# PABannier/bark.cpp

Hardware: NVIDIA H100
Metric: audio sec/sec (inverse RTF), bark-small f16, batch 1 per GPU, semantic->coarse->fine->encodec (higher is better)
Workload: dtype f16 weights/operands, f32 accumulate (reference arithmetic)

## Files before the change

bark.cpp_b200/__init__.py:

```python
from __future__ import annotations

import ctypes as C
import os

import numpy as np

_HERE = os.path.dirname(os.path.abspath(__file__))
LIB_PATH = os.path.join(_HERE, "libbark_b200.so")

PROGRESS_CB = C.CFUNCTYPE(None, C.c_void_p, C.c_int, C.c_int, C.c_void_p)


class BarkContextParams(C.Structure):
    _fields_ = [
        ("verbosity", C.c_int), ("temp", C.c_float), ("fine_temp", C.c_float), ("min_eos_p", C.c_float),
        ("sliding_window_size", C.c_int32), ("max_coarse_history", C.c_int32), ("sample_rate", C.c_int32),
        ("target_bandwidth", C.c_int32), ("cls_token_id", C.c_int32), ("sep_token_id", C.c_int32),
        ("n_steps_text_encoder", C.c_int32), ("text_pad_token", C.c_int32), ("text_encoding_offset", C.c_int32),
        ("semantic_rate_hz", C.c_float), ("semantic_pad_token", C.c_int32), ("semantic_vocab_size", C.c_int32),
        ("semantic_infer_token", C.c_int32), ("coarse_rate_hz", C.c_float), ("coarse_infer_token", C.c_int32),
        ("coarse_semantic_pad_token", C.c_int32), ("n_coarse_codebooks", C.c_int32), ("n_fine_codebooks", C.c_int32),
        ("codebook_size", C.c_int32), ("progress_callback", PROGRESS_CB), ("progress_callback_user_data", C.c_void_p),
    ]


class BarkStatistics(C.Structure):
    _fields_ = [("t_load_us", C.c_int64), ("t_eval_us", C.c_int64), ("t_semantic_us", C.c_int64), ("t_coarse_us", C.c_int64),
                ("t_fine_us", C.c_int64), ("n_sample_semantic", C.c_int32), ("n_sample_coarse", C.c_int32), ("n_sample_fine", C.c_int32)]


EXPORTS = [
    "bark_context_default_params", "bark_load_model", "bark_generate_audio", "bark_get_audio_data", "bark_get_audio_data_size",
    "bark_get_load_time", "bark_get_eval_time", "bark_reset_statistics", "bark_model_quantize", "bark_free",
    "bark_b200_set_device", "bark_b200_version", "bark_b200_gpt_eval", "bark_b200_fine_eval", "bark_b200_encodec_decode",
    "bark_b200_sample", "bark_b200_sample_rows", "bark_b200_reseed", "bark_b200_tokenize", "bark_b200_forward_text_encoder",
    "bark_b200_forward_coarse_encoder", "bark_b200_forward_fine_encoder", "bark_b200_get_tokens", "bark_b200_set_tokens",
    "bark_b200_get_stats", "bark_b200_get_hparams", "bark_b200_kernel_launches", "bark_b200_layernorm_fallbacks",
    "bark_b200_profile_enable", "bark_b200_profile_report", "bark_b200_io_counters", "bark_b200_decode_timing",
    "bark_b200_shard_init", "bark_b200_shard_connect", "bark_b200_shard_nvlink_bytes",
    "bark_b200_fast_mode", "bark_b200_fast_gemm", "bark_b200_fast_attention", "bark_b200_parity_attention",
    "bark_b200_generate_batch", "bark_b200_batch_audio", "bark_b200_batch_tokens", "bark_b200_gpt_eval_slot", "bark_b200_gpt_step_batch",
    "ggml_time_init", "ggml_time_us", "ggml_time_ms", "ggml_init", "ggml_free",
]

_lib = None


def lib() -> C.CDLL:
    global _lib
    if _lib is not None:
        return _lib
    if not os.path.exists(LIB_PATH):
        raise RuntimeError(f"{LIB_PATH} is missing: build the CUDA extension first (python -c 'import __graft_entry__ as g; g.build()'). "
                           "There is no CPU fallback.")
    L = C.CDLL(LIB_PATH)
    vp, i32p, f32p = C.c_void_p, C.c_void_p, C.c_void_p
    L.bark_context_default_params.restype = BarkContextParams
    L.bark_load_model.restype = vp
    L.bark_load_model.argtypes = [C.c_char_p, BarkContextParams, C.c_uint32]
    L.bark_generate_audio.restype = C.c_bool
    L.bark_generate_audio.argtypes = [vp, C.c_char_p, C.c_int]
    L.bark_get_audio_data.restype = C.POINTER(C.c_float)
    L.bark_get_audio_data.argtypes = [vp]
# ... 31 lines not shown
    L.bark_b200_kernel_launches.restype = C.c_ulonglong
    L.bark_b200_layernorm_fallbacks.restype = C.c_uint
    L.bark_b200_layernorm_fallbacks.argtypes = [vp]
    L.bark_b200_profile_enable.argtypes = [C.c_int]
    L.bark_b200_profile_report.restype = C.c_int
    L.bark_b200_profile_report.argtypes = [C.c_char_p, C.c_int]
    L.bark_b200_io_counters.argtypes = [C.POINTER(C.c_ulonglong), C.POINTER(C.c_ulonglong), C.c_int]
    L.bark_b200_decode_timing.restype = C.c_int
    L.bark_b200_decode_timing.argtypes = [vp, C.c_void_p, C.c_int]
    L.bark_b200_shard_init.restype = C.c_int
    L.bark_b200_shard_init.argtypes = [vp, C.c_int, C.c_int, vp]
    L.bark_b200_shard_connect.restype = C.c_int
    L.bark_b200_shard_connect.argtypes = [vp, vp]
    L.bark_b200_shard_nvlink_bytes.restype = C.c_ulonglong
    L.bark_b200_shard_nvlink_bytes.argtypes = [vp, C.c_int]
    L.bark_b200_fast_mode.restype = C.c_int
    L.bark_b200_fast_mode.argtypes = [vp]
    L.bark_b200_fast_gemm.restype = C.c_int
    L.bark_b200_fast_gemm.argtypes = [vp, vp, vp, C.c_int, C.c_int, C.c_int, C.c_int, C.c_int]
    L.bark_b200_fast_attention.restype = C.c_int
    L.bark_b200_fast_attention.argtypes = [vp, vp, vp, vp, C.c_int, C.c_int, C.c_int]
    L.bark_b200_parity_attention.restype = C.c_int
    L.bark_b200_parity_attention.argtypes = [vp, vp, vp, vp] + [C.c_int] * 7
    L.bark_b200_generate_batch.restype = C.c_bool
    L.bark_b200_generate_batch.argtypes = [vp, C.POINTER(C.c_char_p), C.POINTER(C.c_uint32), C.c_int, C.c_int]
    L.bark_b200_batch_audio.restype = C.c_int
    L.bark_b200_batch_audio.argtypes = [vp, C.c_int, f32p, C.c_int]
    L.bark_b200_batch_tokens.restype = C.c_int
    L.bark_b200_batch_tokens.argtypes = [vp, C.c_int, C.c_int, i32p, C.c_int]
    L.bark_b200_gpt_eval_slot.restype = C.c_int
    L.bark_b200_gpt_eval_slot.argtypes = [vp, C.c_int, C.c_int, i32p, C.c_int, C.POINTER(C.c_int), C.c_int, f32p]
    L.bark_b200_gpt_step_batch.restype = C.c_int
    L.bark_b200_gpt_step_batch.argtypes = [vp, C.c_int, C.c_int, i32p, i32p, i32p, f32p]
    L.ggml_time_us.restype = C.c_int64
    _lib = L
    return L


def _p(a: np.ndarray):
    return a.ctypes.data_as(C.c_void_p)


class Bark:

    def __init__(self, model_path: str, seed: int = 0, n_steps_text_encoder: int | None = None, temp=None, fine_temp=None,
                 min_eos_p=None, device: int | None = None, progress=None):
# ... 212 lines not shown
def fast_attention(q: np.ndarray, k: np.ndarray, v: np.ndarray, n_head: int) -> np.ndarray:
    q, k, v = (np.ascontiguousarray(a, np.float16) for a in (q, k, v))
    n, E = q.shape
    out = np.zeros((n, E), np.float16)
    if not lib().bark_b200_fast_attention(_p(q), _p(k), _p(v), _p(out), n, E, n_head):
        raise RuntimeError("bark_b200_fast_attention failed")
    return out


ATTN_PATHS = {"auto": 0, "fused": 1, "tiled": 2}


def parity_attention(q: np.ndarray, k: np.ndarray, v: np.ndarray, n_head: int, n_past: int = 0, causal: bool = False, path: str = "auto") -> np.ndarray:
    q, k, v = (np.ascontiguousarray(a, np.float32) for a in (q, k, v))
    N, E = q.shape
    n_kv = k.shape[0]
    assert k.shape == v.shape == (n_kv, E), (q.shape, k.shape, v.shape)
    out = np.zeros((N, E), np.float32)
    if not lib().bark_b200_parity_attention(_p(q), _p(k), _p(v), _p(out), N, n_kv, n_past, E, n_head, int(causal), ATTN_PATHS[path]):
        raise RuntimeError("bark_b200_parity_attention failed")
    return out


def kernel_launches() -> int:
    return int(lib().bark_b200_kernel_launches())


def profile_enable(on: bool):
    lib().bark_b200_profile_enable(int(on))


def profile_report() -> dict:
    import json
    n = lib().bark_b200_profile_report(None, 0)
    buf = C.create_string_buffer(n + 16)
    lib().bark_b200_profile_report(buf, n + 16)
    return json.loads(buf.value.decode())


def io_counters(reset: bool = False):
    a, b = C.c_ulonglong(0), C.c_ulonglong(0)
    lib().bark_b200_io_counters(C.byref(a), C.byref(b), int(reset))
    return a.value, b.value
```

bark.cpp_b200/csrc/bark_api.cu:

```cuda
#include "../../include/bark_b200.h"
#include "context.h"
#include "gpt_kernels.h"

#include <algorithm>
#include <cmath>
#include <cstring>

using namespace bark;

namespace {

thread_local int g_device_override = -1;
bool quiet() { static const bool q = [] { const char * e = getenv("BARK_B200_QUIET"); return e && *e && *e != '0'; }(); return q; }

inline bool is_alpha(unsigned char c) { return (c >= 'a' && c <= 'z') || (c >= 'A' && c <= 'Z'); }
inline bool is_digit(unsigned char c) { return c >= '0' && c <= '9'; }
inline bool is_punct(unsigned char c) { return c > 32 && c < 127 && !is_alpha(c) && !is_digit(c); }

char fold_accent(unsigned char second) {
    const unsigned cp = 0xC0u + (second - 0x80u);
    const bool lower = cp >= 0xE0;
    const unsigned up = lower ? cp - 0x20 : cp;
    char base = 0;
    if (up >= 0xC0 && up <= 0xC5) base = 'A';
// ... 916 lines not shown
    BARK_CUDA_CHECK(cudaMalloc(&dq, (size_t) N * E * 4)); BARK_CUDA_CHECK(cudaMalloc(&dk, (size_t) n_kv * E * 4));
    BARK_CUDA_CHECK(cudaMalloc(&dv, (size_t) n_kv * E * 4)); BARK_CUDA_CHECK(cudaMalloc(&dout, (size_t) N * E * 4));
    BARK_CUDA_CHECK(cudaMalloc(&dsc, (size_t) H * N * n_kv * 4));
    BARK_CUDA_CHECK(cudaMemcpy(dq, q, (size_t) N * E * 4, cudaMemcpyHostToDevice)); BARK_CUDA_CHECK(cudaMemcpy(dk, k, (size_t) n_kv * E * 4, cudaMemcpyHostToDevice));
    BARK_CUDA_CHECK(cudaMemcpy(dv, v, (size_t) n_kv * E * 4, cudaMemcpyHostToDevice));
    BARK_CUDA_CHECK(cudaMemset(dout, 0xff, (size_t) N * E * 4));
    if (path == ATTN_TILED) {
        int dev = 0, n_sm = 0;
        BARK_CUDA_CHECK(cudaGetDevice(&dev)); BARK_CUDA_CHECK(cudaDeviceGetAttribute(&n_sm, cudaDevAttrMultiProcessorCount, dev));
        if (N > attn_tiled_max_rows(H, n_sm)) return 0;
    }
    attention(dq, dk, dv, N, n_kv, n_past, E, H, causal != 0, dsc, dout, W_Q4_0, E, 0, (AttnPath) path);
    BARK_CUDA_CHECK(cudaGetLastError());
    const cudaError_t e = cudaDeviceSynchronize();
    if (e != cudaSuccess) { fprintf(stderr, "bark_b200_parity_attention: %s\n", cudaGetErrorString(e)); return 0; }
    BARK_CUDA_CHECK(cudaMemcpy(out, dout, (size_t) N * E * 4, cudaMemcpyDeviceToHost));
    return 1;
}
extern "C" int bark_b200_parity_attention(const float * q, const float * k, const float * v, float * out, int N, int n_kv, int n_past, int E, int H, int causal,
                                          int path) {
    return guarded((int) 0, [&] { return bark_b200_parity_attention_impl(q, k, v, out, N, n_kv, n_past, E, H, causal, path); });
}

extern "C" bool bark_b200_generate_batch(struct bark_context * ctx, const char * const * texts, const uint32_t * seeds, int n, int n_threads) {
    (void) n_threads;
    return guarded(false, [&] { return generate_batch(ctx, texts, seeds, n); });
}
extern "C" int bark_b200_batch_audio(struct bark_context * ctx, int i, float * out, int cap) {
    if (!ctx || i < 0 || i >= (int) ctx->batch.results.size()) return -1;
    const std::vector<float> & a = ctx->batch.results[(size_t) i].audio;
    if (out) memcpy(out, a.data(), sizeof(float) * std::min(a.size(), (size_t) std::max(cap, 0)));
    return (int) a.size();
}
extern "C" int bark_b200_batch_tokens(struct bark_context * ctx, int i, int stage, int32_t * out, int cap) {
    if (!ctx || i < 0 || i >= (int) ctx->batch.results.size()) return -1;
    return copy_tokens(ctx->batch.results[(size_t) i], stage, out, cap);
}
static int bark_b200_gpt_eval_slot_impl(struct bark_context * ctx, int which, int slot, const int32_t * tokens, int n, int * n_past, int merge_ctx, float * logits_out) {
    if (!ctx || which < 0 || which > 1 || slot < 0 || slot >= kMaxBatch || !tokens || !n_past || !logits_out) return 0;
    BARK_CUDA_CHECK(cudaSetDevice(ctx->device));
    if (!ensure_batch_slots(ctx, slot + 1)) return 0;
    return gpt_eval(ctx, *pick(ctx, which), tokens, n, n_past, merge_ctx != 0, logits_out, 0, 0, ctx->batch.k[which][slot], ctx->batch.v[which][slot]) ? 1 : 0;
}
extern "C" int bark_b200_gpt_eval_slot(struct bark_context * ctx, int which, int slot, const int32_t * tokens, int n, int * n_past, int merge_ctx, float * logits_out) {
    return guarded((int) 0, [&] { return bark_b200_gpt_eval_slot_impl(ctx, which, slot, tokens, n, n_past, merge_ctx, logits_out); });
}
// ... 26 lines not shown
```

bark.cpp_b200/csrc/gemm_kernels.cu:

```cuda
#include "epilogue.cuh"
#include "gpt_kernels.h"

#include <algorithm>
#include <string.h>

namespace bark {

namespace {

__device__ __forceinline__ uint32_t smem_u32(const void * p) { return (uint32_t) __cvta_generic_to_shared(p); }
__device__ __forceinline__ void mbar_init(uint32_t bar, uint32_t count) { asm volatile("mbarrier.init.shared::cta.b64 [%0], %1;" ::"r"(bar), "r"(count)); }
__device__ __forceinline__ void mbar_expect_tx(uint32_t bar, uint32_t bytes) { asm volatile("mbarrier.arrive.expect_tx.shared::cta.b64 _, [%0], %1;" ::"r"(bar), "r"(bytes) : "memory"); }
__device__ __forceinline__ void mbar_wait(uint32_t bar, uint32_t parity) {
    asm volatile(
        "{\n\t.reg .pred p;\n\t"
        "WAIT_%=:\n\t"
        "mbarrier.try_wait.parity.shared::cta.b64 p, [%0], %1;\n\t"
        "@p bra DONE_%=;\n\t"
        "bra WAIT_%=;\n\t"
        "DONE_%=:\n\t}" ::"r"(bar), "r"(parity) : "memory");
}
__device__ __forceinline__ void mbar_arrive(uint32_t bar) { asm volatile("mbarrier.arrive.shared::cta.b64 _, [%0];" ::"r"(bar) : "memory"); }
__device__ __forceinline__ void tma_bulk_g2s(uint32_t dst, const void * src, uint32_t bytes, uint32_t bar) {
    asm volatile("cp.async.bulk.shared::cluster.global.mbarrier::complete_tx::bytes [%0], [%1], %2, [%3];" ::"r"(dst), "l"(src), "r"(bytes), "r"(bar) : "memory");
}

template <int N, int MASK>
__device__ __forceinline__ void butterfly_stage(float (&r)[64], bool upper) {
#pragma unroll
    for (int i = 0; i < N / 2; i++) {
        const float keep = upper ? r[i + N / 2] : r[i];
        const float send = upper ? r[i] : r[i + N / 2];
        r[i] = __fadd_rn(keep, __shfl_xor_sync(0xffffffffu, send, MASK));
    }
}
__device__ __forceinline__ int butterfly_reduce64(float (&r)[64], int lane) {
    butterfly_stage<64, 16>(r, (lane & 16) != 0);
    butterfly_stage<32, 8>(r, (lane & 8) != 0);
    butterfly_stage<16, 4>(r, (lane & 4) != 0);
    butterfly_stage<8, 1>(r, (lane & 1) != 0);
    butterfly_stage<4, 2>(r, (lane & 2) != 0);
    return ((lane & 16) << 1) | ((lane & 8) << 1) | ((lane & 4) << 1) | ((lane & 1) << 2) | (lane & 2);
}

constexpr int kBM = 32, kBO = 16, kStages = 4;
constexpr int kStageBytes = (kBM + kBO) * 512;

template <typename T> struct QuadOp;
template <> struct QuadOp<__half> {
    typedef uint2 V;
    static constexpr int kGroupsPerStage = 2;
    __device__ __forceinline__ static float elem(const uint2 & u, int c) {
        const uint32_t w = c < 2 ? u.x : u.y;
        const __half2 h = *reinterpret_cast<const __half2 *>(&w);
        return (c & 1) ? __high2float(h) : __low2float(h);
    }
};
template <> struct QuadOp<float> {
    typedef uint4 V;
    static constexpr int kGroupsPerStage = 1;
    __device__ __forceinline__ static float elem(const uint4 & u, int c) { return __uint_as_float(c == 0 ? u.x : c == 1 ? u.y : c == 2 ? u.z : u.w); }
};

}

template <typename T>
__global__ void __launch_bounds__(256, 2) lane_gemm_tiled_kernel(const T * __restrict__ Wg, int K, int w_gs, int O, const T * __restrict__ act, int act_gs, int M, MatmulEpilogue ep) {
    typedef typename QuadOp<T>::V QV;
    constexpr int GPS = QuadOp<T>::kGroupsPerStage;
    constexpr int kRowB = kGmGroup * sizeof(T);
    extern __shared__ __align__(128) unsigned char smem[];
    const uint32_t full = smem_u32(smem + kStages * kStageBytes);
    int * const cnt = reinterpret_cast<int *>(smem + kStages * kStageBytes + kStages * 8);
    const int tid = threadIdx.x, lane = tid & 31, warp = tid >> 5;
    const int wm = warp >> 1, wo = warp & 1;
    const int nsteps = K >> 5;
    const int ngroups = (nsteps + 3) >> 2;
    const int nstages = (ngroups + GPS - 1) / GPS;
    const int tiles_o = (O + kBO - 1) / kBO, tiles_m = (M + kBM - 1) / kBM, n_tiles = tiles_o * tiles_m;
    const int my_tiles = ((int) blockIdx.x < n_tiles) ? (n_tiles - 1 - (int) blockIdx.x) / (int) gridDim.x + 1 : 0;
    const int total_steps = my_tiles * nstages;

    if (tid == 0) {
        for (int s = 0; s < kStages; s++) { mbar_init(full + s * 8, 1); cnt[s] = 0; }
        asm volatile("fence.mbarrier_init.release.cluster;" ::: "memory");
    }
    __syncthreads();
    auto issue = [&](int step) {
        const int ti = step / nstages, sg = step - ti * nstages;
        const int tile = blockIdx.x + ti * gridDim.x;
        const int m0 = (tile / tiles_o) * kBM, o0 = (tile % tiles_o) * kBO;
        const int slot = step % kStages;
        const uint32_t bar = full + slot * 8;
        const int g0 = sg * GPS, ng = min(GPS, ngroups - g0);
        mbar_expect_tx(bar, (uint32_t)(ng * (kBM + kBO) * kRowB));
        const uint32_t dst = smem_u32(smem + (size_t) slot * kStageBytes);
        for (int j = 0; j < ng; j++) {
            tma_bulk_g2s(dst + j * (kBM + kBO) * kRowB, act + (size_t)(g0 + j) * act_gs + (size_t) m0 * kGmGroup, kBM * kRowB, bar);
            tma_bulk_g2s(dst + j * (kBM + kBO) * kRowB + kBM * kRowB, Wg + (size_t)(g0 + j) * w_gs + (size_t) o0 * kGmGroup, kBO * kRowB, bar);
        }
    };
    if (tid == 0) for (int s0 = 0; s0 < kStages && s0 < total_steps; s0++) issue(s0);

    int step = 0;
    for (int ti = 0; ti < my_tiles; ti++) {
        const int tile = blockIdx.x + ti * gridDim.x;
        const int m0 = (tile / tiles_o) * kBM, o0 = (tile % tiles_o) * kBO;
        float acc[64];
#pragma unroll
        for (int i = 0; i < 64; i++) acc[i] = 0.0f;
        for (int sg = 0; sg < nstages; sg++, step++) {
            const int slot = step % kStages;
            mbar_wait(full + slot * 8, (uint32_t)(step / kStages) & 1);
            const unsigned char * st = smem + (size_t) slot * kStageBytes;
#pragma unroll
            for (int j = 0; j < GPS; j++) {
                const int g = sg * GPS + j;
                if (g < ngroups) {
                    const int steps = min(4, nsteps - g * 4);
                    const unsigned char * ga = st + j * (kBM + kBO) * kRowB + lane * sizeof(QV), * gw = ga + kBM * kRowB;
                    QV pa[8], pw[8];
#pragma unroll
                    for (int mi = 0; mi < 8; mi++) pa[mi] = *reinterpret_cast<const QV *>(ga + (wm * 8 + mi) * kRowB);
#pragma unroll
                    for (int oi = 0; oi < 8; oi++) pw[oi] = *reinterpret_cast<const QV *>(gw + (wo * 8 + oi) * kRowB);
#pragma unroll
                    for (int c = 0; c < 4; c++) {
                        if (c < steps) {
                            float af[8], wf[8];
#pragma unroll
                            for (int mi = 0; mi < 8; mi++) af[mi] = QuadOp<T>::elem(pa[mi], c);
#pragma unroll
                            for (int oi = 0; oi < 8; oi++) wf[oi] = QuadOp<T>::elem(pw[oi], c);
#pragma unroll
                            for (int mi = 0; mi < 8; mi++)
#pragma unroll
                                for (int oi = 0; oi < 8; oi++) acc[mi * 8 + oi] = __fmaf_rn(wf[oi], af[mi], acc[mi * 8 + oi]);
                        }
                    }
                }
            }
            __syncwarp();
            if (lane == 0) {
                __threadfence_block();
                if (atomicAdd_block(&cnt[slot], 1) == 7) {
                    cnt[slot] = 0;
                    __threadfence_block();
                    asm volatile("fence.proxy.async.shared::cta;" ::: "memory");
                    if (step + kStages < total_steps) issue(step + kStages);
                }
            }
        }
        const int base = butterfly_reduce64(acc, lane);
        const int m = m0 + wm * 8 + (base >> 3), o = o0 + wo * 8 + (base & 7);
        if (m < M) {
            if (o < O) matmul_epilogue(ep, m, o, acc[0]);
            if (o + 1 < O) matmul_epilogue(ep, m, o + 1, acc[1]);
        }
    }
}

void lane_gemm_tiled(const DMat & W, const void * act, int act_gs, int rows, const MatmulEpilogue & ep, cudaStream_t s) {
    const size_t smem = (size_t) kStages * kStageBytes + kStages * 8 + kStages * 4 + 64;
    int dev = 0, n_sm = 0;
    BARK_CUDA_CHECK(cudaGetDevice(&dev));
    BARK_CUDA_CHECK(cudaDeviceGetAttribute(&n_sm, cudaDevAttrMultiProcessorCount, dev));
    static std::atomic<unsigned long long> configured{0};
    if (first_use_on_this_device(configured)) {
        BARK_CUDA_CHECK(cudaFuncSetAttribute(lane_gemm_tiled_kernel<__half>, cudaFuncAttributeMaxDynamicSharedMemorySize, (int) smem));
        BARK_CUDA_CHECK(cudaFuncSetAttribute(lane_gemm_tiled_kernel<float>, cudaFuncAttributeMaxDynamicSharedMemorySize, (int) smem));
    }
    if (!W.p_gm) { fprintf(stderr, "bark_b200: matrix has no group-major copy for the tiled mat-mul\n"); throw std::runtime_error("unsupported configuration (see the message above)"); }
    const int n_tiles = ((W.n_out + kBO - 1) / kBO) * ((rows + kBM - 1) / kBM);
    const int grid = min(n_tiles, 2 * n_sm);
    const int w_gs = W.o_pad * kGmGroup;
    if (W.type == W_F16) BARK_LAUNCH((lane_gemm_tiled_kernel<__half>), grid, 256, smem, s, (const __half *) W.p_gm, W.K, w_gs, W.n_out, (const __half *) act, act_gs, rows, ep);
    else                 BARK_LAUNCH((lane_gemm_tiled_kernel<float>), grid, 256, smem, s, (const float *) W.p_gm, W.K, w_gs, W.n_out, (const float *) act, act_gs, rows, ep);
}

constexpr int kAttnQ = 32, kAttnKT = 64, kAttnVK = 512, kAttnVW = 16;
constexpr int kAttnVLd = kAttnVW + 4;

__host__ __device__ inline int attn_ld(int n_kv) { return ((n_kv + 31) & ~31) + 1; }
__host__ __device__ inline int attn_ring_off(int n_kv) { return (kAttnQ * attn_ld(n_kv) + 3) & ~3; }

namespace {
__device__ __forceinline__ void cp_async_16(void * dst, const float * src) { asm volatile("cp.async.cg.shared.global [%0], [%1], 16;" ::"r"(smem_u32(dst)), "l"(src) : "memory"); }
__device__ __forceinline__ void cp_async_commit() { asm volatile("cp.async.commit_group;" ::: "memory"); }
__device__ __forceinline__ void cp_async_wait_prev() { asm volatile("cp.async.wait_group 1;" ::: "memory"); }
}

template <int DSTEPS>
__global__ void __launch_bounds__(256, 1) attn_fused_kernel(const float * __restrict__ Q, const float * __restrict__ Kc, const float * __restrict__ Vc,
                                                            int N, int n_kv, int n_past, int E, float scale, int causal,
                                                            void * __restrict__ act, int wt, int Kp) {
    constexpr int D = DSTEPS * 32;
    extern __shared__ __align__(16) float sm[];
    const int tid = threadIdx.x, lane = tid & 31, warp = tid >> 5;
    const int h = blockIdx.y, q0 = blockIdx.x * kAttnQ;
    const int ld = attn_ld(n_kv);
// ... 239 lines not shown
```

bark.cpp_b200/csrc/gpt_kernels.h:

```cpp
#pragma once
#include "model.h"

namespace bark {

enum EpiMode : int { EPI_STORE = 0, EPI_RESID = 1, EPI_GELU_ACT = 2, EPI_QKV = 3 };

struct MatmulEpilogue {
    int mode = EPI_STORE;
    float * out = nullptr; int ldo = 0;
    float * k_out = nullptr, * v_out = nullptr;
    int n_peer = 0; float * k_peer[7] = {nullptr}, * v_peer[7] = {nullptr};
    void * act_out = nullptr; int act_wt = 0, act_Kp = 0;
    const __half * gelu_tab = nullptr;
};

void permute_to_li(const void * src_rowmajor, void * dst_li, int n_out, int K, WType t, cudaStream_t s);
void permute_to_gm(const void * src_rowmajor, void * dst_gm, int n_out, int o_pad, int K, WType t, cudaStream_t s);

void gpt_embed_causal(const GPTModel & m, const int32_t * d_tok, int N, int n_past, bool merge, float * x, cudaStream_t s, const int32_t * d_pos = nullptr);
void gpt_embed_fine(const GPTModel & m, const int32_t * d_ids, int nn, float * x, cudaStream_t s, int row0 = 0, int rows = 1024);

void layernorm_act(const float * x, int rows, int E, const float * g, const float * b, void * act, WType wt, int Kp,
                   unsigned * fallback_counter, cudaStream_t s);

void lane_matmul(const DMat & W, const void * act, int act_gs, int rows, const MatmulEpilogue & ep, cudaStream_t s);

enum AttnPath : int { ATTN_AUTO = 0, ATTN_FUSED = 1, ATTN_TILED = 2 };
int  attn_tiled_max_rows(int H, int n_sm);
void attention(const float * Q, const float * Kc, const float * Vc, int N, int n_kv, int n_past, int E, int H, bool causal,
               float * scores, void * act, WType wt, int Kp, cudaStream_t s, AttnPath path = ATTN_AUTO);

struct BatchKV { float * k[8], * v[8]; };
void attention_batch(const float * Q, const float * Kst, const float * Vst, const BatchKV & kv, const int32_t * d_pos, int B, int max_kv, int E, int H,
                     float * scores, void * act, WType wt, int Kp, cudaStream_t s);

void q4_split(const void * raw_blocks, size_t n_blocks, void * qs, void * scales, cudaStream_t s);
void q4_set_scratch(void * q8, void * q8_scales);
void q4_matmul(const DMat & W, const void * act_f32, int ld_act, int rows, const MatmulEpilogue & ep, cudaStream_t s);

bool   qx_supported(WType t);
size_t qx_block_bytes(WType t);
void   qx_split(const void * raw_blocks, size_t n_blocks, WType t, void * qs, void * qh, void * d, void * m, cudaStream_t s);
void   qx_set_scratch(void * q8, void * q8_scales, void * q8_sums);
void   qx_embed_causal(const GPTModel & m, const int32_t * d_tok, int N, int n_past, bool merge, float * x, cudaStream_t s, const int32_t * d_pos);
void   qx_embed_fine(const GPTModel & m, const int32_t * d_ids, int nn, float * x, cudaStream_t s);
void   qx_matmul(const DMat & W, const void * act_f32, int ld_act, int rows, const MatmulEpilogue & ep, cudaStream_t s);

void lane_gemm_tiled(const DMat & W, const void * act, int act_gs, int rows, const MatmulEpilogue & ep, cudaStream_t s);

enum { FEPI_F32 = 0, FEPI_RESID = 1, FEPI_GELU16 = 2, FEPI_QKV16 = 4 };
struct FastEpi {
    int mode = FEPI_F32;
    float * out32 = nullptr; __half * out16 = nullptr; int ldo = 0;
    __half * vt = nullptr; int vt_ld = 0, v_col0 = 0;
};
int  fast_gemm(const __half * A, int lda, const __half * W, int ldw, int M, int N, int K, const FastEpi & ep, int n_sm, int bn, cudaStream_t s);
bool fast_attention(const __half * qk, int ldq, int k_col0, const __half * vt, int n, int E, int H, __half * out, cudaStream_t s);
void fast_layernorm(const float * x, int rows, int E, const float * g, const float * b, __half * out, cudaStream_t s);

constexpr int kDecodeReplicas = 8;
struct DecodePhase { const void * w; int n_out, row_bytes, K, pad; const void * ws; };
struct DecodeLayerVec { const float * ln_1_g, * ln_1_b, * ln_2_g, * ln_2_b; };
struct DecodeArgs {
    const DecodePhase * phases;
    const DecodeLayerVec * layer_vecs;
    const void * wte; const float * wpe; const float * ln_f_g, * ln_f_b; const __half * gelu_tab;
    float * mem_k, * mem_v;
    unsigned long long * gx, * gq, * gk, * gv, * gatt, * gff, * gscores;
    float * logits;
    unsigned tag_base; unsigned * ln_fallbacks;
    unsigned long long * timing;
// ... 13 lines not shown
```

bark.cpp_b200/csrc/loader.cu:

```cuda
#include "context.h"
#include "codec_kernels.h"
#include "gpt_kernels.h"

#include <cmath>
#include <cstring>
#include <fstream>

namespace bark {

static const uint32_t kMagic = 0x67676d6c;

void * ctx_alloc(bark_context * ctx, size_t bytes) {
    void * p = nullptr;
    BARK_CUDA_CHECK(cudaMalloc(&p, bytes ? bytes : 16));
    ctx->device_allocs.push_back(p);
    return p;
}

namespace {

template <typename T> bool rd(std::ifstream & f, T & v) { f.read(reinterpret_cast<char *>(&v), sizeof(T)); return (bool) f; }

size_t type_bytes(int ttype, size_t nel) {
    switch (ttype) {
// ... 105 lines not shown
                const size_t n_blocks = h.nel / 32;
                d.n_out = s.ne1; d.K = s.ne0; d.Kp = d.K; d.type = m.wtype;
                d.p = ctx_alloc(ctx, n_blocks * (m.wtype == W_Q8_0 ? 32 : 16)); d.scales = ctx_alloc(ctx, n_blocks * 2);
                d.mins = ctx_alloc(ctx, n_blocks * 2); d.qh = ctx_alloc(ctx, n_blocks * 4);
                qx_split(raw, n_blocks, m.wtype, d.p, d.qh, d.scales, d.mins, ctx->stream);
                BARK_CUDA_CHECK(cudaStreamSynchronize(ctx->stream));
                BARK_CUDA_CHECK(cudaFree(raw));
                continue;
            }
            if (m.wtype == W_Q4_0) {
                const size_t n_blocks = h.nel / 32;
                d.n_out = s.ne1; d.K = s.ne0; d.Kp = d.K; d.type = W_Q4_0;
                d.p = ctx_alloc(ctx, n_blocks * 16); d.scales = ctx_alloc(ctx, n_blocks * 2);
                q4_split(raw, n_blocks, d.p, d.scales, ctx->stream);
                BARK_CUDA_CHECK(cudaStreamSynchronize(ctx->stream));
                BARK_CUDA_CHECK(cudaFree(raw));
                if (ctx->params.verbosity == HIGH) printf("%48s - [%5d, %5d], type = %d, %6.2f MB\n", h.name.c_str(), h.ne[0], h.ne[1], h.ttype, bytes / 1024.0 / 1024.0);
                continue;
            }
            d.n_out = s.ne1; d.K = s.ne0; d.type = m.wtype; d.Kp = li_padded_k(d.K, m.wtype == W_F16 ? 2 : 4);
            d.p = ctx_alloc(ctx, (size_t) d.n_out * d.Kp * (m.wtype == W_F16 ? 2 : 4));
            permute_to_li(raw, d.p, d.n_out, d.K, m.wtype, ctx->stream);
            if (s.gm) {
                d.o_pad = (d.n_out + 15) / 16 * 16;
                const size_t gm_bytes = (size_t) gm_groups(d.K) * d.o_pad * kGmGroup * (m.wtype == W_F16 ? 2 : 4);
                d.p_gm = ctx_alloc(ctx, gm_bytes);
                permute_to_gm(raw, d.p_gm, d.n_out, d.o_pad, d.K, m.wtype, ctx->stream);
            }
            BARK_CUDA_CHECK(cudaStreamSynchronize(ctx->stream));
            if (ctx->fast_mode && !causal && m.wtype == W_F16) { d.p_rm = raw; ctx->device_allocs.push_back(raw); }
            else BARK_CUDA_CHECK(cudaFree(raw));
        } else {
            void * raw = upload_raw(ctx, f, bytes, host, true);
            if (!raw) return false;
            if (s.kind == Slot::TABLE) *s.table = raw; else *s.vec = (float *) raw;
        }
        if (ctx->params.verbosity == HIGH) printf("%48s - [%5d, %5d], type = %d, %6.2f MB\n", h.name.c_str(), h.ne[0], h.ne[1], h.ttype, bytes / 1024.0 / 1024.0);
    }
    for (auto & kv : slots) {
        const Slot & s = kv.second;
        const bool present = s.kind == Slot::MATRIX ? s.mat->p != nullptr : s.kind == Slot::TABLE ? *s.table != nullptr : *s.vec != nullptr;
        if (!present) { fprintf(stderr, "%s: tensor '%s' missing from the %s model\n", __func__, kv.first.c_str(), what); return false; }
    }
    if (causal) {
        const size_t n = (size_t) m.n_layer * m.block_size * E;
        m.mem_k = (float *) ctx_alloc(ctx, n * 4); m.mem_v = (float *) ctx_alloc(ctx, n * 4);
        BARK_CUDA_CHECK(cudaMemsetAsync(m.mem_k, 0, n * 4, ctx->stream)); BARK_CUDA_CHECK(cudaMemsetAsync(m.mem_v, 0, n * 4, ctx->stream));
// ... 157 lines not shown
```

include/bark_b200.h:

```cpp
#pragma once
#include "bark.h"

#ifdef __cplusplus
extern "C" {
#endif

BARK_API void bark_b200_set_device(int cuda_device);
BARK_API const char * bark_b200_version(void);

BARK_API int  bark_b200_gpt_eval(struct bark_context * ctx, int which, const int32_t * tokens, int n, int * n_past, int merge_ctx, float * logits_out);
BARK_API int  bark_b200_fine_eval(struct bark_context * ctx, const int32_t * in_buffer, int nn, float * logits_out);
BARK_API int  bark_b200_encodec_decode(struct bark_context * ctx, const int32_t * codes, int n_frames, float * out, int out_cap);
BARK_API int  bark_b200_sample(struct bark_context * ctx, int which, const float * logits, int n, float temp, float * eos_p);
BARK_API int  bark_b200_sample_rows(struct bark_context * ctx, const float * logits , int n, int rows, float temp, int32_t * tokens_out,
                                     float * eos_p_out );
BARK_API void bark_b200_reseed(struct bark_context * ctx, uint32_t seed);
BARK_API void bark_b200_tokenize(struct bark_context * ctx, const char * text, int32_t * out513);

BARK_API bool bark_b200_forward_text_encoder(struct bark_context * ctx, int n_threads);
BARK_API bool bark_b200_forward_coarse_encoder(struct bark_context * ctx, int n_threads);
BARK_API bool bark_b200_forward_fine_encoder(struct bark_context * ctx, int n_threads);

BARK_API int  bark_b200_get_tokens(struct bark_context * ctx, int stage, int32_t * out, int cap);
BARK_API void bark_b200_set_tokens(struct bark_context * ctx, int stage, const int32_t * in, int n);
// ... 5 lines not shown
BARK_API void bark_b200_profile_enable(int on);
BARK_API int  bark_b200_profile_report(char * buf, int cap);
BARK_API void bark_b200_io_counters(unsigned long long * h2d_bytes, unsigned long long * d2h_bytes, int reset);
BARK_API int  bark_b200_decode_timing(struct bark_context * ctx, unsigned long long * out, int n);


BARK_API int  bark_b200_shard_init(struct bark_context * ctx, int rank, int world, void * handle_out);
BARK_API int  bark_b200_shard_connect(struct bark_context * ctx, const void * all_handles);
BARK_API unsigned long long bark_b200_shard_nvlink_bytes(struct bark_context * ctx, int reset);

BARK_API bool bark_b200_generate_batch(struct bark_context * ctx, const char * const * texts, const uint32_t * seeds, int n, int n_threads);
BARK_API int  bark_b200_batch_audio(struct bark_context * ctx, int i, float * out, int cap);
BARK_API int  bark_b200_batch_tokens(struct bark_context * ctx, int i, int stage, int32_t * out, int cap);
BARK_API int  bark_b200_gpt_eval_slot(struct bark_context * ctx, int which, int slot, const int32_t * tokens, int n, int * n_past, int merge_ctx, float * logits_out);
BARK_API int  bark_b200_gpt_step_batch(struct bark_context * ctx, int which, int B, const int32_t * slots, const int32_t * tokens, int * n_past, float * logits_out);

BARK_API int  bark_b200_fast_mode(struct bark_context * ctx);
BARK_API int  bark_b200_fast_gemm(const uint16_t * A, const uint16_t * W, void * C, int M, int N, int K, int epilogue, int bn);
BARK_API int  bark_b200_fast_attention(const uint16_t * q, const uint16_t * k, const uint16_t * v, uint16_t * out, int n, int E, int H);

BARK_API int  bark_b200_parity_attention(const float * q, const float * k, const float * v, float * out, int N, int n_kv, int n_past, int E, int H, int causal,
                                         int path);

#ifdef __cplusplus
}
#endif
```

Measured before the change: 12.24.

## Templatize tiled GEMM; add 32x32 f16 tile with register pipelining and smem reduce

```diff
diff --git a/bark.cpp_b200/__init__.py b/bark.cpp_b200/__init__.py
--- a/bark.cpp_b200/__init__.py
+++ b/bark.cpp_b200/__init__.py
@@ -38,7 +38,7 @@
     "bark_b200_get_stats", "bark_b200_get_hparams", "bark_b200_kernel_launches", "bark_b200_layernorm_fallbacks",
     "bark_b200_profile_enable", "bark_b200_profile_report", "bark_b200_io_counters", "bark_b200_decode_timing",
     "bark_b200_shard_init", "bark_b200_shard_connect", "bark_b200_shard_nvlink_bytes",
-    "bark_b200_fast_mode", "bark_b200_fast_gemm", "bark_b200_fast_attention", "bark_b200_parity_attention",
+    "bark_b200_fast_mode", "bark_b200_fast_gemm", "bark_b200_fast_attention", "bark_b200_parity_attention", "bark_b200_parity_gemm",
     "bark_b200_generate_batch", "bark_b200_batch_audio", "bark_b200_batch_tokens", "bark_b200_gpt_eval_slot", "bark_b200_gpt_step_batch",
     "ggml_time_init", "ggml_time_us", "ggml_time_ms", "ggml_init", "ggml_free",
 ]
@@ -116,6 +116,8 @@
     L.bark_b200_fast_attention.argtypes = [vp, vp, vp, vp, C.c_int, C.c_int, C.c_int]
     L.bark_b200_parity_attention.restype = C.c_int
     L.bark_b200_parity_attention.argtypes = [vp, vp, vp, vp] + [C.c_int] * 7
+    L.bark_b200_parity_gemm.restype = C.c_int
+    L.bark_b200_parity_gemm.argtypes = [vp, vp, vp] + [C.c_int] * 6 + [vp]
     L.bark_b200_generate_batch.restype = C.c_bool
     L.bark_b200_generate_batch.argtypes = [vp, C.POINTER(C.c_char_p), C.POINTER(C.c_uint32), C.c_int, C.c_int]
     L.bark_b200_batch_audio.restype = C.c_int
@@ -374,6 +376,36 @@
     return out
 
 
+PARITY_EPILOGUES = {"store": 0, "resid": 1, "gelu": 2, "qkv": 3}
+
+
+def parity_gemm(A: np.ndarray, W: np.ndarray, epilogue: str = "store", variant: int = 0, resid: np.ndarray | None = None,
+                gelu_tab: np.ndarray | None = None, return_variant: bool = False):
+    dt = np.float16 if np.asarray(A).dtype == np.float16 else np.float32
+    A = np.ascontiguousarray(A, dt); W = np.ascontiguousarray(W, dt)
+    M, K = A.shape; N = W.shape[0]
+    assert W.shape[1] == K, (A.shape, W.shape)
+    if epilogue == "resid":
+        out = np.array(resid, np.float32, order="C", copy=True)
+        assert out.shape == (M, N), out.shape
+    else:
+        out = np.zeros((M, N), dt if epilogue == "gelu" else np.float32)
+    tab = None
+    if epilogue == "gelu":
+        tab = np.ascontiguousarray(gelu_tab, np.uint16)
+        assert tab.shape == (65536,), tab.shape
+    r = lib().bark_b200_parity_gemm(_p(A), _p(W), _p(out), M, N, K, 1 if dt == np.float16 else 0, PARITY_EPILOGUES[epilogue], variant,
+                                    None if tab is None else _p(tab))
+    if r == -1:
+        raise GuardBandError(f"bark_b200_parity_gemm ({epilogue}, {M}x{N}x{K}, variant {variant}) wrote outside its output")
+    if r <= 0:
+        raise RuntimeError(f"bark_b200_parity_gemm ({epilogue}, {M}x{N}x{K}, variant {variant}) failed")
+    if epilogue == "qkv":
+        flat = out.reshape(-1)
+        out = tuple(flat[i * M * (N // 3):(i + 1) * M * (N // 3)].reshape(M, N // 3) for i in range(3))
+    return (out, r) if return_variant else out
+
+
 def kernel_launches() -> int:
     return int(lib().bark_b200_kernel_launches())
 
diff --git a/bark.cpp_b200/csrc/bark_api.cu b/bark.cpp_b200/csrc/bark_api.cu
--- a/bark.cpp_b200/csrc/bark_api.cu
+++ b/bark.cpp_b200/csrc/bark_api.cu
@@ -962,6 +962,67 @@
     return guarded((int) 0, [&] { return bark_b200_parity_attention_impl(q, k, v, out, N, n_kv, n_past, E, H, causal, path); });
 }
 
+static int bark_b200_parity_gemm_impl(const void * A, const void * W, void * C, int M, int N, int K, int wtype, int epilogue, int variant,
+                                      const uint16_t * gelu_tab) {
+    if (!A || !W || !C || M < 1 || N < 1 || K < 32 || K % 32 || (wtype != W_F32 && wtype != W_F16) || variant < 0) return 0;
+    if (epilogue < EPI_STORE || epilogue > EPI_QKV || (epilogue == EPI_QKV && N % 3) || (epilogue == EPI_GELU_ACT && !gelu_tab)) return 0;
+    constexpr size_t kGuard = 4096;
+    constexpr unsigned char kPattern = 0x5a;
+    const size_t es = wtype == W_F16 ? 2 : 4;
+    const int rows_cap = (M + 31) / 32 * 32, o_pad = (N + kGemmOPad - 1) / kGemmOPad * kGemmOPad;
+    const size_t a_bytes = (size_t) gm_groups(K) * rows_cap * kGmGroup * es, w_bytes = (size_t) gm_groups(K) * o_pad * kGmGroup * es;
+    const size_t out_bytes = epilogue == EPI_GELU_ACT ? (size_t) gm_groups(N) * rows_cap * kGmGroup * es : (size_t) M * N * 4;
+    struct Buffers {
+        void * p[6] = {nullptr, nullptr, nullptr, nullptr, nullptr, nullptr};
+        ~Buffers() { for (void * b : p) cudaFree(b); }
+    } d;
+    void *& d_rm = d.p[0], *& d_a = d.p[1], *& d_w = d.p[2], *& d_out = d.p[3], *& d_tab = d.p[4];
+    BARK_CUDA_CHECK(cudaMalloc(&d_rm, (size_t) std::max(M, N) * K * es));
+    BARK_CUDA_CHECK(cudaMalloc(&d_a, a_bytes)); BARK_CUDA_CHECK(cudaMalloc(&d_w, w_bytes));
+    BARK_CUDA_CHECK(cudaMemcpy(d_rm, A, (size_t) M * K * es, cudaMemcpyHostToDevice));
+    permute_to_gm(d_rm, d_a, M, rows_cap, K, (WType) wtype, 0);
+    BARK_CUDA_CHECK(cudaStreamSynchronize(0));
+    BARK_CUDA_CHECK(cudaMemcpy(d_rm, W, (size_t) N * K * es, cudaMemcpyHostToDevice));
+    permute_to_gm(d_rm, d_w, N, o_pad, K, (WType) wtype, 0);
+    BARK_CUDA_CHECK(cudaMalloc(&d_out, out_bytes + 2 * kGuard));
+    unsigned char * const reg = (unsigned char *) d_out;
+    BARK_CUDA_CHECK(cudaMemset(reg, kPattern, out_bytes + 2 * kGuard));
+    if (epilogue == EPI_RESID) BARK_CUDA_CHECK(cudaMemcpy(reg + kGuard, C, out_bytes, cudaMemcpyHostToDevice));
+    else                       BARK_CUDA_CHECK(cudaMemset(reg + kGuard, 0xff, out_bytes));
+    DMat dm; dm.n_out = N; dm.K = K; dm.type = (WType) wtype; dm.p_gm = d_w; dm.o_pad = o_pad;
+    MatmulEpilogue ep; ep.mode = epilogue;
+    float * const out = (float *)(reg + kGuard);
+    if (epilogue == EPI_STORE || epilogue == EPI_RESID) { ep.out = out; ep.ldo = N; }
+    else if (epilogue == EPI_QKV) { const int E = N / 3; ep.out = out; ep.k_out = out + (size_t) M * E; ep.v_out = out + 2 * (size_t) M * E; ep.ldo = E; }
+    else {
+        BARK_CUDA_CHECK(cudaMalloc(&d_tab, 65536 * 2));
+        BARK_CUDA_CHECK(cudaMemcpy(d_tab, gelu_tab, 65536 * 2, cudaMemcpyHostToDevice));
+        ep.act_out = out; ep.act_wt = wtype; ep.act_Kp = rows_cap * kGmGroup; ep.gelu_tab = (const __half *) d_tab;
+    }
+    const int ran = lane_gemm_tiled(dm, d_a, rows_cap * kGmGroup, M, ep, 0, variant);
+    BARK_CUDA_CHECK(cudaGetLastError());
+    const cudaError_t e = cudaDeviceSynchronize();
+    if (e != cudaSuccess) { fprintf(stderr, "bark_b200_parity_gemm: %s\n", cudaGetErrorString(e)); return 0; }
+    if (!ran) return 0;
+    std::vector<unsigned char> h(out_bytes + 2 * kGuard);
+    BARK_CUDA_CHECK(cudaMemcpy(h.data(), reg, h.size(), cudaMemcpyDeviceToHost));
+    bool guards_intact = true;
+    for (size_t i = 0; i < kGuard; i++) guards_intact &= h[i] == kPattern && h[kGuard + out_bytes + i] == kPattern;
+    if (!guards_intact) { fprintf(stderr, "bark_b200_parity_gemm: a store landed outside the output (guard band overwritten)\n"); return -1; }
+    const unsigned char * o = h.data() + kGuard;
+    if (epilogue != EPI_GELU_ACT) memcpy(C, o, out_bytes);
+    else {
+        const size_t gs = (size_t) rows_cap * kGmGroup;
+        for (int m = 0; m < M; m++)
+            for (int k = 0; k < N; k++) memcpy((unsigned char *) C + ((size_t) m * N + k) * es, o + gm_offset(m, k, gs) * es, es);
+    }
+    return ran;
+}
+extern "C" int bark_b200_parity_gemm(const void * A, const void * W, void * C, int M, int N, int K, int wtype, int epilogue, int variant,
+                                     const uint16_t * gelu_tab) {
+    return guarded((int) 0, [&] { return bark_b200_parity_gemm_impl(A, W, C, M, N, K, wtype, epilogue, variant, gelu_tab); });
+}
+
 extern "C" bool bark_b200_generate_batch(struct bark_context * ctx, const char * const * texts, const uint32_t * seeds, int n, int n_threads) {
     (void) n_threads;
     return guarded(false, [&] { return generate_batch(ctx, texts, seeds, n); });
diff --git a/bark.cpp_b200/csrc/gemm_kernels.cu b/bark.cpp_b200/csrc/gemm_kernels.cu
--- a/bark.cpp_b200/csrc/gemm_kernels.cu
+++ b/bark.cpp_b200/csrc/gemm_kernels.cu
@@ -20,7 +20,11 @@
         "bra WAIT_%=;\n\t"
         "DONE_%=:\n\t}" ::"r"(bar), "r"(parity) : "memory");
 }
-__device__ __forceinline__ void mbar_arrive(uint32_t bar) { asm volatile("mbarrier.arrive.shared::cta.b64 _, [%0];" ::"r"(bar) : "memory"); }
+__device__ __forceinline__ int atom_add_acq_rel_cta(int * p, int v) {
+    int old;
+    asm volatile("atom.acq_rel.cta.shared::cta.add.u32 %0, [%1], %2;" : "=r"(old) : "r"(smem_u32(p)), "r"(v) : "memory");
+    return old;
+}
 __device__ __forceinline__ void tma_bulk_g2s(uint32_t dst, const void * src, uint32_t bytes, uint32_t bar) {
     asm volatile("cp.async.bulk.shared::cluster.global.mbarrier::complete_tx::bytes [%0], [%1], %2, [%3];" ::"r"(dst), "l"(src), "r"(bytes), "r"(bar) : "memory");
 }
@@ -43,8 +47,20 @@
     return ((lane & 16) << 1) | ((lane & 8) << 1) | ((lane & 4) << 1) | ((lane & 1) << 2) | (lane & 2);
 }
 
-constexpr int kBM = 32, kBO = 16, kStages = 4;
-constexpr int kStageBytes = (kBM + kBO) * 512;
+constexpr int kStages = 4;
+constexpr int kRedLd = 36;
+
+template <int WM_, int WO_, int OT_, int MINB_, bool PIPE_ = false> struct TileCfg {
+    static constexpr int WM = WM_, WO = WO_, OT = OT_, MINB = MINB_;
+    static constexpr bool PIPE = PIPE_;
+    static constexpr int kWarps = WM * WO, kThreads = 32 * kWarps, kBM = 8 * WM, kBO = OT * WO, kNAcc = 8 * OT;
+    static constexpr int kStageBytes = (kBM + kBO) * 512;
+    static constexpr bool kSmemReduce = MINB == 1;
+    static constexpr size_t kRedOff = ((size_t) kStages * kStageBytes + kStages * 12 + 15) & ~(size_t) 15;
+    static constexpr size_t kSmem = kRedOff + (kSmemReduce ? (size_t) kWarps * 32 * kRedLd * 4 : 0);
+};
+typedef TileCfg<4, 2, 8, 2>  Tile32x16;
+typedef TileCfg<4, 4, 8, 1, true> Tile32x32;
 
 template <typename T> struct QuadOp;
 template <> struct QuadOp<__half> {
@@ -62,18 +78,65 @@
     __device__ __forceinline__ static float elem(const uint4 & u, int c) { return __uint_as_float(c == 0 ? u.x : c == 1 ? u.y : c == 2 ? u.z : u.w); }
 };
 
-}
-
-template <typename T>
-__global__ void __launch_bounds__(256, 2) lane_gemm_tiled_kernel(const T * __restrict__ Wg, int K, int w_gs, int O, const T * __restrict__ act, int act_gs, int M, MatmulEpilogue ep) {
+template <typename T, int OT, bool FULL>
+__device__ __forceinline__ void fma_group(const unsigned char * ga, const unsigned char * gw, float (&acc)[8 * OT], int steps) {
     typedef typename QuadOp<T>::V QV;
-    constexpr int GPS = QuadOp<T>::kGroupsPerStage;
+    constexpr int kRowB = kGmGroup * sizeof(T);
+    QV pa[8], pw[OT];
+#pragma unroll
+    for (int mi = 0; mi < 8; mi++) pa[mi] = *reinterpret_cast<const QV *>(ga + mi * kRowB);
+#pragma unroll
+    for (int oi = 0; oi < OT; oi++) pw[oi] = *reinterpret_cast<const QV *>(gw + oi * kRowB);
+#pragma unroll
+    for (int c = 0; c < 4; c++) {
+        if (FULL || c < steps) {
+            float af[8], wf[OT];
+#pragma unroll
+            for (int mi = 0; mi < 8; mi++) af[mi] = QuadOp<T>::elem(pa[mi], c);
+#pragma unroll
+            for (int oi = 0; oi < OT; oi++) wf[oi] = QuadOp<T>::elem(pw[oi], c);
+#pragma unroll
+            for (int mi = 0; mi < 8; mi++)
+#pragma unroll
+                for (int oi = 0; oi < OT; oi++) acc[mi * OT + oi] = __fmaf_rn(wf[oi], af[mi], acc[mi * OT + oi]);
+        }
+    }
+}
+
+template <int OT>
+__device__ __forceinline__ void fma_half(const uint32_t (&a)[8], const uint32_t (&w)[OT], float (&acc)[8 * OT]) {
+#pragma unroll
+    for (int c = 0; c < 2; c++) {
+        float af[8], wf[OT];
+#pragma unroll
+        for (int mi = 0; mi < 8; mi++) { const __half2 h = *reinterpret_cast<const __half2 *>(&a[mi]); af[mi] = c ? __high2float(h) : __low2float(h); }
+#pragma unroll
+        for (int oi = 0; oi < OT; oi++) { const __half2 h = *reinterpret_cast<const __half2 *>(&w[oi]); wf[oi] = c ? __high2float(h) : __low2float(h); }
+#pragma unroll
+        for (int mi = 0; mi < 8; mi++)
+#pragma unroll
+            for (int oi = 0; oi < OT; oi++) acc[mi * OT + oi] = __fmaf_rn(wf[oi], af[mi], acc[mi * OT + oi]);
+    }
+}
+template <int OT>
+__device__ __forceinline__ void load_half(const unsigned char * ga, const unsigned char * gw, int h, uint32_t (&a)[8], uint32_t (&w)[OT]) {
+#pragma unroll
+    for (int mi = 0; mi < 8; mi++) a[mi] = *reinterpret_cast<const uint32_t *>(ga + mi * 256 + h * 4);
+#pragma unroll
+    for (int oi = 0; oi < OT; oi++) w[oi] = *reinterpret_cast<const uint32_t *>(gw + oi * 256 + h * 4);
+}
+
+}
+
+template <typename T, typename Cfg>
+__global__ void __launch_bounds__(Cfg::kThreads, Cfg::MINB) lane_gemm_tiled_kernel(const T * __restrict__ Wg, int K, int w_gs, int O, const T * __restrict__ act, int act_gs, int M, MatmulEpilogue ep) {
+    constexpr int GPS = QuadOp<T>::kGroupsPerStage, OT = Cfg::OT, kBM = Cfg::kBM, kBO = Cfg::kBO, kStageBytes = Cfg::kStageBytes;
     constexpr int kRowB = kGmGroup * sizeof(T);
     extern __shared__ __align__(128) unsigned char smem[];
     const uint32_t full = smem_u32(smem + kStages * kStageBytes);
     int * const cnt = reinterpret_cast<int *>(smem + kStages * kStageBytes + kStages * 8);
     const int tid = threadIdx.x, lane = tid & 31, warp = tid >> 5;
-    const int wm = warp >> 1, wo = warp & 1;
+    const int wm = warp / Cfg::WO, wo = warp % Cfg::WO;
     const int nsteps = K >> 5;
     const int ngroups = (nsteps + 3) >> 2;
     const int nstages = (ngroups + GPS - 1) / GPS;
@@ -106,76 +169,107 @@
     for (int ti = 0; ti < my_tiles; ti++) {
         const int tile = blockIdx.x + ti * gridDim.x;
         const int m0 = (tile / tiles_o) * kBM, o0 = (tile % tiles_o) * kBO;
-        float acc[64];
-#pragma unroll
-        for (int i = 0; i < 64; i++) acc[i] = 0.0f;
+        float acc[Cfg::kNAcc];
+#pragma unroll
+        for (int i = 0; i < Cfg::kNAcc; i++) acc[i] = 0.0f;
         for (int sg = 0; sg < nstages; sg++, step++) {
             const int slot = step % kStages;
             mbar_wait(full + slot * 8, (uint32_t)(step / kStages) & 1);
             const unsigned char * st = smem + (size_t) slot * kStageBytes;
+            const unsigned char * const ga0 = st + lane * sizeof(typename QuadOp<T>::V) + wm * 8 * kRowB;
+            const unsigned char * const gw0 = st + kBM * kRowB + lane * sizeof(typename QuadOp<T>::V) + wo * OT * kRowB;
+            if constexpr (Cfg::PIPE) {
+                if (nsteps - sg * GPS * 4 >= GPS * 4) {
+                    uint32_t a0[8], w0[OT], a1[8], w1[OT];
+                    load_half<OT>(ga0, gw0, 0, a0, w0);
+#pragma unroll
+                    for (int j = 0; j < GPS; j++) {
+                        const int off = j * (kBM + kBO) * kRowB;
+                        load_half<OT>(ga0 + off, gw0 + off, 1, a1, w1);
+                        fma_half<OT>(a0, w0, acc);
+                        if (j + 1 < GPS) load_half<OT>(ga0 + off + (kBM + kBO) * kRowB, gw0 + off + (kBM + kBO) * kRowB, 0, a0, w0);
+                        fma_half<OT>(a1, w1, acc);
+                    }
+                    goto released;
+                }
+            }
 #pragma unroll
             for (int j = 0; j < GPS; j++) {
                 const int g = sg * GPS + j;
                 if (g < ngroups) {
-                    const int steps = min(4, nsteps - g * 4);
-                    const unsigned char * ga = st + j * (kBM + kBO) * kRowB + lane * sizeof(QV), * gw = ga + kBM * kRowB;
-                    QV pa[8], pw[8];
-#pragma unroll
-                    for (int mi = 0; mi < 8; mi++) pa[mi] = *reinterpret_cast<const QV *>(ga + (wm * 8 + mi) * kRowB);
-#pragma unroll
-                    for (int oi = 0; oi < 8; oi++) pw[oi] = *reinterpret_cast<const QV *>(gw + (wo * 8 + oi) * kRowB);
-#pragma unroll
-                    for (int c = 0; c < 4; c++) {
-                        if (c < steps) {
-                            float af[8], wf[8];
-#pragma unroll
-                            for (int mi = 0; mi < 8; mi++) af[mi] = QuadOp<T>::elem(pa[mi], c);
-#pragma unroll
-                            for (int oi = 0; oi < 8; oi++) wf[oi] = QuadOp<T>::elem(pw[oi], c);
-#pragma unroll
-                            for (int mi = 0; mi < 8; mi++)
-#pragma unroll
-                                for (int oi = 0; oi < 8; oi++) acc[mi * 8 + oi] = __fmaf_rn(wf[oi], af[mi], acc[mi * 8 + oi]);
-                        }
-                    }
+                    const unsigned char * ga = ga0 + j * (kBM + kBO) * kRowB, * gw = gw0 + j * (kBM + kBO) * kRowB;
+                    const int steps = nsteps - g * 4;
+                    if (steps >= 4) fma_group<T, OT, true>(ga, gw, acc, 4);
+                    else            fma_group<T, OT, false>(ga, gw, acc, steps);
                 }
             }
+        released:
             __syncwarp();
             if (lane == 0) {
-                __threadfence_block();
-                if (atomicAdd_block(&cnt[slot], 1) == 7) {
-                    cnt[slot] = 0;
-                    __threadfence_block();
+                if ((atom_add_acq_rel_cta(&cnt[slot], 1) + 1) % Cfg::kWarps == 0) {
                     asm volatile("fence.proxy.async.shared::cta;" ::: "memory");
                     if (step + kStages < total_steps) issue(step + kStages);
                 }
             }
         }
-        const int base = butterfly_reduce64(acc, lane);
-        const int m = m0 + wm * 8 + (base >> 3), o = o0 + wo * 8 + (base & 7);
-        if (m < M) {
-            if (o < O) matmul_epilogue(ep, m, o, acc[0]);
-            if (o + 1 < O) matmul_epilogue(ep, m, o + 1, acc[1]);
-        }
-    }
-}
-
-void lane_gemm_tiled(const DMat & W, const void * act, int act_gs, int rows, const MatmulEpilogue & ep, cudaStream_t s) {
-    const size_t smem = (size_t) kStages * kStageBytes + kStages * 8 + kStages * 4 + 64;
+        if constexpr (Cfg::kSmemReduce) {
+            float * const red = reinterpret_cast<float *>(smem + Cfg::kRedOff) + warp * 32 * kRedLd;
+#pragma unroll
+            for (int sl = 0; sl < Cfg::kNAcc / 32; sl++) {
+                __syncwarp();
+#pragma unroll
+                for (int j = 0; j < 32; j++) red[j * kRedLd + lane] = acc[sl * 32 + j];
+                __syncwarp();
+                float a[32];
+#pragma unroll
+                for (int q = 0; q < 8; q++) {
+                    const float4 t = *reinterpret_cast<const float4 *>(red + lane * kRedLd + q * 4);
+                    a[4 * q] = t.x; a[4 * q + 1] = t.y; a[4 * q + 2] = t.z; a[4 * q + 3] = t.w;
+                }
+                const int i = sl * 32 + lane;
+                const int m = m0 + wm * 8 + i / OT, o = o0 + wo * OT + i % OT;
+                const float r = lane_tree_reduce_local(a);
+                if (m < M && o < O) matmul_epilogue(ep, m, o, r);
+            }
+        } else {
+            static_assert(Cfg::kNAcc == 64, "the butterfly combines 64 outputs");
+            const int base = butterfly_reduce64(acc, lane);
+            const int m = m0 + wm * 8 + (base >> 3), o = o0 + wo * 8 + (base & 7);
+            if (m < M) {
+                if (o < O) matmul_epilogue(ep, m, o, acc[0]);
+                if (o + 1 < O) matmul_epilogue(ep, m, o + 1, acc[1]);
+            }
+        }
+    }
+}
+
+template <typename T, typename Cfg>
+static void launch_tiled(const DMat & W, const void * act, int act_gs, int rows, const MatmulEpilogue & ep, int n_sm, cudaStream_t s) {
+    static std::atomic<unsigned long long> configured{0};
+    if (first_use_on_this_device(configured))
+        BARK_CUDA_CHECK(cudaFuncSetAttribute(lane_gemm_tiled_kernel<T, Cfg>, cudaFuncAttributeMaxDynamicSharedMemorySize, (int) Cfg::kSmem));
+    const int n_tiles = ((W.n_out + Cfg::kBO - 1) / Cfg::kBO) * ((rows + Cfg::kBM - 1) / Cfg::kBM);
+    const int grid = min(n_tiles, Cfg::MINB * n_sm);
+    BARK_LAUNCH((lane_gemm_tiled_kernel<T, Cfg>), grid, Cfg::kThreads, Cfg::kSmem, s, (const T *) W.p_gm, W.K, W.o_pad * kGmGroup, W.n_out,
+                (const T *) act, act_gs, rows, ep);
+}
+
+int lane_gemm_tiled(const DMat & W, const void * act, int act_gs, int rows, const MatmulEpilogue & ep, cudaStream_t s, int variant) {
+    if (!W.p_gm) { fprintf(stderr, "bark_b200: matrix has no group-major copy for the tiled mat-mul\n"); throw std::runtime_error("unsupported configuration (see the message above)"); }
+    if (W.o_pad % kGemmOPad) { fprintf(stderr, "bark_b200: group-major rows padded to %d, need a multiple of %d\n", W.o_pad, kGemmOPad); throw std::runtime_error("unsupported configuration (see the message above)"); }
     int dev = 0, n_sm = 0;
     BARK_CUDA_CHECK(cudaGetDevice(&dev));
     BARK_CUDA_CHECK(cudaDeviceGetAttribute(&n_sm, cudaDevAttrMultiProcessorCount, dev));
-    static std::atomic<unsigned long long> configured{0};
-    if (first_use_on_this_device(configured)) {
-        BARK_CUDA_CHECK(cudaFuncSetAttribute(lane_gemm_tiled_kernel<__half>, cudaFuncAttributeMaxDynamicSharedMemorySize, (int) smem));
-        BARK_CUDA_CHECK(cudaFuncSetAttribute(lane_gemm_tiled_kernel<float>, cudaFuncAttributeMaxDynamicSharedMemorySize, (int) smem));
-    }
-    if (!W.p_gm) { fprintf(stderr, "bark_b200: matrix has no group-major copy for the tiled mat-mul\n"); throw std::runtime_error("unsupported configuration (see the message above)"); }
-    const int n_tiles = ((W.n_out + kBO - 1) / kBO) * ((rows + kBM - 1) / kBM);
-    const int grid = min(n_tiles, 2 * n_sm);
-    const int w_gs = W.o_pad * kGmGroup;
-    if (W.type == W_F16) BARK_LAUNCH((lane_gemm_tiled_kernel<__half>), grid, 256, smem, s, (const __half *) W.p_gm, W.K, w_gs, W.n_out, (const __half *) act, act_gs, rows, ep);
-    else                 BARK_LAUNCH((lane_gemm_tiled_kernel<float>), grid, 256, smem, s, (const float *) W.p_gm, W.K, w_gs, W.n_out, (const float *) act, act_gs, rows, ep);
+    if (variant == 0) variant = W.type == W_F16 ? 2 : 1;
+    if (W.type == W_F16) {
+        if (variant == 1) launch_tiled<__half, Tile32x16>(W, act, act_gs, rows, ep, n_sm, s);
+        else if (variant == 2) launch_tiled<__half, Tile32x32>(W, act, act_gs, rows, ep, n_sm, s);
+        else return 0;
+    } else if (W.type == W_F32) {
+        if (variant == 1) launch_tiled<float, Tile32x16>(W, act, act_gs, rows, ep, n_sm, s);
+        else return 0;
+    } else return 0;
+    return variant;
 }
 
 constexpr int kAttnQ = 32, kAttnKT = 64, kAttnVK = 512, kAttnVW = 16;
diff --git a/bark.cpp_b200/csrc/gpt_kernels.h b/bark.cpp_b200/csrc/gpt_kernels.h
--- a/bark.cpp_b200/csrc/gpt_kernels.h
+++ b/bark.cpp_b200/csrc/gpt_kernels.h
@@ -46,7 +46,8 @@
 void   qx_embed_fine(const GPTModel & m, const int32_t * d_ids, int nn, float * x, cudaStream_t s);
 void   qx_matmul(const DMat & W, const void * act_f32, int ld_act, int rows, const MatmulEpilogue & ep, cudaStream_t s);
 
-void lane_gemm_tiled(const DMat & W, const void * act, int act_gs, int rows, const MatmulEpilogue & ep, cudaStream_t s);
+constexpr int kGemmOPad = 32;
+int lane_gemm_tiled(const DMat & W, const void * act, int act_gs, int rows, const MatmulEpilogue & ep, cudaStream_t s, int variant = 0);
 
 enum { FEPI_F32 = 0, FEPI_RESID = 1, FEPI_GELU16 = 2, FEPI_QKV16 = 4 };
 struct FastEpi {
diff --git a/bark.cpp_b200/csrc/loader.cu b/bark.cpp_b200/csrc/loader.cu
--- a/bark.cpp_b200/csrc/loader.cu
+++ b/bark.cpp_b200/csrc/loader.cu
@@ -151,7 +151,7 @@
             d.p = ctx_alloc(ctx, (size_t) d.n_out * d.Kp * (m.wtype == W_F16 ? 2 : 4));
             permute_to_li(raw, d.p, d.n_out, d.K, m.wtype, ctx->stream);
             if (s.gm) {
-                d.o_pad = (d.n_out + 15) / 16 * 16;
+                d.o_pad = (d.n_out + kGemmOPad - 1) / kGemmOPad * kGemmOPad;
                 const size_t gm_bytes = (size_t) gm_groups(d.K) * d.o_pad * kGmGroup * (m.wtype == W_F16 ? 2 : 4);
                 d.p_gm = ctx_alloc(ctx, gm_bytes);
                 permute_to_gm(raw, d.p_gm, d.n_out, d.o_pad, d.K, m.wtype, ctx->stream);
diff --git a/include/bark_b200.h b/include/bark_b200.h
--- a/include/bark_b200.h
+++ b/include/bark_b200.h
@@ -51,6 +51,9 @@
 BARK_API int  bark_b200_parity_attention(const float * q, const float * k, const float * v, float * out, int N, int n_kv, int n_past, int E, int H, int causal,
                                          int path);
 
+BARK_API int  bark_b200_parity_gemm(const void * A, const void * W, void * C, int M, int N, int K, int wtype, int epilogue, int variant,
+                                    const uint16_t * gelu_tab);
+
 #ifdef __cplusplus
 }
 #endif
```

Result: faster. 12.74 (median of 6 runs) (+4.1%).
